# andres-quintela/manette

Hardware: AMD Instinct MI355X
Metric: env-steps/sec (ec x t_max frames per update) (higher is better)
Workload: dtype fp32

## Files before the change

manette_amd/csrc/net.hip:

```cpp
#include <string>
#include <vector>
#include <cmath>
#include <algorithm>
#include <tuple>

#include "gemm.h"
#include "jobs.h"
#include "trunk_fused.h"
#include "nips_bwd.h"
#include "dconv.h"
#include "nature_bwd.h"

namespace mt {

template <int C>
struct NipsArch {
  using Layers = std::tuple<ConvGeom<C, 16, 8, 4, 84, 84, false>, ConvGeom<16, 32, 4, 2, 20, 20, false>>;
  static constexpr int NCONV = 2;
  static constexpr unsigned POOL = 0;
  static constexpr int FLAT = 9 * 9 * 32;
  static constexpr int F = 256;
  static constexpr const char *FC = "fc3";
  static constexpr int FUSED_SLABS = FusedNips<C>::FC_SPLITS;
  static constexpr int FC_ROWS = 0;
// ... 918 lines not shown
                           float alpha) {
  using T = TileConvDgrad<G>;
  if constexpr (PhaseGeom<G>::OK) {
    constexpr int S2 = G::S * G::S;
    const int mp = cdiv(B * PhaseGeom<G>::HQ * PhaseGeom<G>::WQ, T::BM) * T::BM;
    return gemm_job<T>(LdConvBwdAPhase<G>{dY, mp, B}, LdConvBwdBPhase<G>{Wt, mp / T::BM},
                       EpMaskedPhase<G>{dX, Xact, mp, B, act, alpha}, S2 * mp, G::CIN, PhaseGeom<G>::KP, 1);
  } else {
    return gemm_job<T>(LdConvBwdA<G>{dY}, LdConvBwdB<G>{Wt}, EpMasked{dX, Xact, G::CIN, act, alpha},
                       B * G::H * G::W, G::CIN, G::KH * G::KW * G::COUT, 1);
  }
}

template <class G, class GJ>
static auto conv_dgrad_unpool_job(const float *dY, const float *Wt, const float *Pj, const uint8_t *argj,
                                  float *dactj, int B, int act, float alpha) {
  using T = TileConvDgrad<G>;
  static_assert(!PhaseGeom<G>::OK, "pooled inputs feed stride-1 convs (networks.py:206-225)");
  return gemm_job<T>(LdConvBwdA<G>{dY}, LdConvBwdB<G>{Wt}, EpMaskedUnpool<GJ>{dactj, Pj, argj, act, alpha},
                     B * G::H * G::W, G::CIN, G::KH * G::KW * G::COUT, 1);
}

#define MT_TRY(x)              \
  do {                         \
    int rc_ = (x);             \
    if (rc_ != MT_OK) return rc_; \
  } while (0)

template <class Ar, int I>
static const float *layer_out(float *ws, const WsLayout &L) {
  return ws + (pooled<Ar, I>() ? L.pool[I] : L.act[I]);
}

struct FwdExtras {
  const StackSrc *st = nullptr;
  uint32_t *sync = nullptr;
};

template <class Ar, int I = 0>
static int trunk_forward(const mt_net *n, const float *P, const void *x, int B, float *ws,
                         const WsLayout &L, hipStream_t s, const FwdExtras &ex = FwdExtras{}) {
  if constexpr (I < Ar::NCONV) {
    using G = LayerG<Ar, I>;
    const float *W = P + n->off_conv[I];
    if (I == 0 && ex.st && !nature_stacking<Ar>() && !frame_stacking<Ar>()) {
      set_error("the stacking conv1 is built for the NIPS, the gray NATURE and the frame (PWYX / LSTM) trunks");
      return MT_ERR_UNSUPPORTED;
    }
    if constexpr (I == 0 && frame_stacking<Ar>()) {
      if (ex.st) {
        if (!ex.sync || x != ex.st->out) {
          set_error("stacking conv1: the input must be the new state rows, with a counter region");
          return MT_ERR_ARG;
        }
        MT_TRY((launch_stack_conv1<G>(*ex.st, W, ws + L.pool[0], (uint8_t *)(ws + L.parg[0]), B, n->cfg.activation,
                                      n->cfg.alpha_leaky, ex.sync, s)));
        return trunk_forward<Ar, 1>(n, P, layer_out<Ar, 0>(ws, L), B, ws, L, s);
      }
    }
    if constexpr (I == 0 && nature_stacking<Ar>()) {
      if (ex.st) {
        if (!ex.sync) {
          set_error("nature chain: no counter region");
          return MT_ERR_ARG;
        }
        return launch_nature_chain<LayerG<Ar, 0>, LayerG<Ar, 1>, LayerG<Ar, 2>>(
            *ex.st, W, P + n->off_conv[1], P + n->off_conv[2], ws + L.act[0], ws + L.act[1], ws + L.act[2], B,
            n->cfg.activation, n->cfg.alpha_leaky, ex.sync, s);
      }
    }
    if constexpr ((G::S == 1 && G::SAME) || (Ar::NCONV == 3 && !G::SAME && G::CIN != 12))
      MT_TRY((conv_forward_direct<G, I == 0, pooled<Ar, I>()>(
          x, W, W + G::KK * G::COUT, ws + (pooled<Ar, I>() ? L.pool[I] : L.act[I]),
          pooled<Ar, I>() ? (uint8_t *)(ws + L.parg[I]) : nullptr, B, n->cfg.activation, n->cfg.alpha_leaky, s)));
    else if constexpr (pooled<Ar, I>())
      MT_TRY((conv_forward_pool<G, I == 0>(x, W, W + G::KK * G::COUT, ws + L.pool[I], (uint8_t *)(ws + L.parg[I]), B,
                                           n->cfg.activation, n->cfg.alpha_leaky, s)));
    else
      MT_TRY((conv_forward<G, I == 0>(x, W, W + G::KK * G::COUT, ws + L.act[I], B, n->cfg.activation,
                                      n->cfg.alpha_leaky, s)));
    return trunk_forward<Ar, I + 1>(n, P, layer_out<Ar, I>(ws, L), B, ws, L, s, ex);
  }
  return MT_OK;
}

struct NormOut {
  float *partials = nullptr;
  size_t n = 0;
};

template <class Ar, int I, class X = NoJob>
static int trunk_backward(const mt_net *n, const float *P, const uint8_t *obs, int B, float *ws,
                          const WsLayout &L, float *grad, hipStream_t s, SlabJob pending = SlabJob{},
                          const NormOut &no = NormOut{}, const X &extra = X{}) {
  using G = LayerG<Ar, I>;
  const int act = n->cfg.activation;
  const float al = n->cfg.alpha_leaky;
  const void *x = I == 0 ? (const void *)obs : (const void *)layer_out<Ar, (I > 0 ? I - 1 : 0)>(ws, L);
  if ((size_t)B * G::H * G::W * G::CIN >= ((size_t)1 << 31)) {
    set_error("batch %d too large for the conv %d weight gradient", B, I);
    return MT_ERR_ARG;
  }
  if ((size_t)B * G::OH * G::OW * G::COUT * 4 >= ((size_t)1 << 31) - 16) {
    set_error("batch %d too large for the conv %d input gradient", B, I);
    return MT_ERR_ARG;
  }
  const auto wg = conv_wgrad_jobs_sel<G, I == 0>(x, ws + L.dact[I], ws + (I % 2 ? L.wslab2 : L.wslab),
                                             grad + n->off_conv[I], B);
  if constexpr (I > 0) {
    constexpr int J = I - 1;
    using GJ = LayerG<Ar, J>;
    if constexpr (pooled<Ar, J>() && G::S == 1 && G::SAME && dconv_bwd_solo<G>()) {
      MT_TRY((conv_dgrad_unpool_solo<G, GJ>(ws + L.dact[I], P + n->off_conv[I], ws + L.pool[J],
                                           (const uint8_t *)(ws + L.parg[J]), ws + L.dact[J], B, act, al, s)));
      MT_TRY(launch_group(s, extra, wg.gemm, pending));
    } else if constexpr (stream_dx<G>()) {
      MT_TRY(launch_group(s, extra, DxStreamJob<G>{ws + L.dact[I], P + n->off_conv[I], ws + L.act[J], ws + L.dact[J], B,
                                            dx_stream_groups<G>(B), act, al},
                          wg.gemm, pending));
    } else if constexpr (pooled<Ar, J>()) {
      MT_TRY(launch_group(s, extra, conv_dgrad_unpool_job<G, GJ>(ws + L.dact[I], P + n->off_conv[I], ws + L.pool[J],
                                                           (const uint8_t *)(ws + L.parg[J]), ws + L.dact[J], B, act,
                                                           al),
                          wg.gemm, pending));
    } else {
      MT_TRY(launch_group(s, extra, conv_dgrad_job<G>(ws + L.dact[I], P + n->off_conv[I], ws + L.act[J], ws + L.dact[J], B,
                                               act, al),
                          wg.gemm, pending));
    }
    return trunk_backward<Ar, J>(n, P, obs, B, ws, L, grad, s, wg.sum, no);
  } else {
    MT_TRY(launch_group(s, extra, wg.gemm, pending));
    SlabJob last = wg.sum;
    if (no.partials && last.blocks() <= MT_NORM_PARTIALS / 2) {
      last.sq = no.partials;
      const size_t b0 = n->off_conv[0], b1 = b0 + last.n;
      SumsqJob rest{grad, no.n, last.blocks() ? b0 : 0, last.blocks() ? b1 : 0, no.partials + last.blocks(),
                    MT_NORM_PARTIALS - last.blocks()};
      return launch_group(s, last, rest);
    }
    MT_TRY(launch_group(s, last));
    if (no.partials)
      return launch_group(s, SumsqJob{grad, no.n, 0, 0, no.partials, MT_NORM_PARTIALS});
    return MT_OK;
  }
}

template <class Ar>
static int nips_conv_backward(const mt_net *n, const float *P, const uint8_t *obs, int B, float *ws,
                              const WsLayout &L, float *grad, hipStream_t s, const NormOut &no) {
  using J = NipsConvBwdJob;
  static_assert(LayerG<Ar, 0>::KK + 1 == 257 && LayerG<Ar, 1>::KK + 1 == 257, "slab rows");
  float *slab1 = ws + L.wslab, *slab2 = ws + L.wslab2;
  MT_TRY(launch_nips_conv_bwd(s, J{obs, ws + L.act[0], ws + L.dact[1], P + n->off_conv[1], ws + L.dact[0], slab1,
                                   slab2, B, n->cfg.activation, n->cfg.alpha_leaky}));
  SlabJob s1{slab1, B, (size_t)J::SLAB1, grad + n->off_conv[0]};
  SlabJob s2{slab2, (B + 1) / 2, (size_t)J::SLAB2, grad + n->off_conv[1]};
  if (!no.partials) return launch_group(s, s1, s2);
  s1.sq = no.partials;
  s2.sq = no.partials + s1.blocks();
  const int used = s1.blocks() + s2.blocks();
  static_assert(MT_NORM_PARTIALS >= 2 * ((257 * 16 / 4 + kSlabCols - 1) / kSlabCols + (257 * 32 / 4 + kSlabCols - 1) / kSlabCols),
                "norm partials");
  return launch_group(s, s1, s2,
                      SumsqJob{grad, no.n, n->off_conv[0], n->off_conv[1] + s2.n, no.partials + used,
                               MT_NORM_PARTIALS - used});
}

template <class Ar, int I = 0>
static void shift_rows(WsLayout &L, size_t row0) {
  if constexpr (I < Ar::NCONV) {
    using G = LayerG<Ar, I>;
    const size_t a = row0 * G::OH * G::OW * G::COUT;
    L.act[I] += a;
    L.dact[I] += a;
    if constexpr (pooled<Ar, I>()) {
      const size_t p = row0 * (G::OH / 2) * (G::OW / 2) * G::COUT;
      L.pool[I] += p;
      L.parg[I] += p / 4;
    }
    shift_rows<Ar, I + 1>(L, row0);
  }
}

struct ActRows {
  float *base;
  WsLayout L;
  size_t h_off;
};
template <class Ar>
static ActRows act_rows(const mt_net *n, float *ws, const WsLayout &L, const TrainRows *tr) {
  if (!tr) return ActRows{ws, L, L.H};
  ActRows a{tr->ws, ws_layout<Ar>(n, tr->rows), 0};
  a.h_off = a.L.H + (size_t)tr->row0 * Ar::F;
  shift_rows<Ar>(a.L, (size_t)tr->row0);
  return a;
}

template <class Ar>
static int forward_impl(const mt_net *n, const float *P, const uint8_t *obs, int B, float *ws,
                        float *v, float *pi, float *rep, const SampleArgs *smp, hipStream_t s,
                        const TrainRows *tr = nullptr, const hipEvent_t *marks = nullptr,
                        const StackSrc *st = nullptr) {
  const WsLayout L = ws_layout<Ar>(n, B);
  const ActRows A = act_rows<Ar>(n, ws, L, tr);
  if (marks) MT_HIP(hipEventRecord(marks[0], s));
  FwdExtras ex;
  ex.st = st;
  ex.sync = reinterpret_cast<uint32_t *>(ws + L.sync);
  MT_TRY((trunk_forward<Ar>(n, P, obs, B, A.base, A.L, s, ex)));
  const float *flat = layer_out<Ar, Ar::NCONV - 1>(A.base, A.L);
  const float *Wfc = P + n->off_fc;
  MT_TRY((launch_fc<Ar>(flat, B, Wfc, ws + L.fcslab, L.fc_splits, s)));
  if (marks) MT_HIP(hipEventRecord(marks[1], s));
  HeadParams hp = head_params(n, P);
  return launch_heads(B, s, ws + L.fcslab, L.fc_splits, B, Wfc + (size_t)Ar::FLAT * Ar::F, n->cfg.activation,
                      n->cfg.alpha_leaky, hp, n->cfg.softmax_temp, A.base + A.h_off, v, pi, rep,
                      smp ? *smp : SampleArgs{});
}

template <class Ar>
static int forward_infer_impl(const mt_net *n, const float *P, const uint8_t *obs, int B, float *ws,
                              float *v, float *pi, float *rep, const SampleArgs *smp, hipStream_t s,
                              const TrainRows *tr = nullptr, const StackSrc *st = nullptr,
                              const hipEvent_t *marks = nullptr) {
  if constexpr (Ar::FUSED_SLABS > 0) {
    constexpr int C = LayerG<Ar, 0>::CIN;
    using Fz = FusedNips<C>;
    const WsLayout L = ws_layout<Ar>(n, B);
    const ActRows A = act_rows<Ar>(n, ws, L, tr);
    const float *Wfc = P + n->off_fc;
    if (marks) MT_HIP(hipEventRecord(marks[0], s));
    MT_TRY((launch_nips_trunk<C>(obs, st, B, P + n->off_conv[0], P + n->off_conv[1], Wfc, n->cfg.activation,
                                 n->cfg.alpha_leaky, A.base + A.L.act[1], tr ? A.base + A.L.act[0] : nullptr,
                                 ws + L.fcslab, s)));
    MT_LAUNCHED();
    if (marks) MT_HIP(hipEventRecord(marks[1], s));
    HeadParams hp = head_params(n, P);
    return launch_heads(B, s, ws + L.fcslab, Fz::FC_SPLITS, B, Wfc + (size_t)Ar::FLAT * Ar::F, n->cfg.activation,
                        n->cfg.alpha_leaky, hp, n->cfg.softmax_temp, A.base + A.h_off, v, pi, rep,
                        smp ? *smp : SampleArgs{});
  } else {
    return forward_impl<Ar>(n, P, obs, B, ws, v, pi, rep, smp, s, tr, marks, st);
  }
}

template <class Ar>
static int forward_boot_impl(const mt_net *n, const float *P, const uint8_t *obs, int B, float *ws, hipStream_t s,
                             const StackSrc *st, uint32_t *advance, uint32_t advance_by) {
  const WsLayout L = ws_layout<Ar>(n, B);
  const float *Wfc = P + n->off_fc;
  if constexpr (Ar::FUSED_SLABS > 0) {
    constexpr int C = LayerG<Ar, 0>::CIN;
    return launch_nips_trunk<C>(obs, st, B, P + n->off_conv[0], P + n->off_conv[1], Wfc, n->cfg.activation,
                                n->cfg.alpha_leaky, ws + L.act[1], nullptr, ws + L.fcslab, s, advance, advance_by);
  } else {
    if (advance && Ar::FC_ROWS == 0) {
      set_error("sequence-base advance: row-split dense layers only");
      return MT_ERR_UNSUPPORTED;
    }
    FwdExtras ex;
    ex.st = st;
    ex.sync = reinterpret_cast<uint32_t *>(ws + L.sync);
    MT_TRY((trunk_forward<Ar>(n, P, obs, B, ws, L, s, ex)));
    return launch_fc<Ar>(layer_out<Ar, Ar::NCONV - 1>(ws, L), B, Wfc, ws + L.fcslab, L.fc_splits, s, advance,
                         advance_by);
  }
}

template <class Ar>
static int loss_bwd_launch(const mt_net *n, const float *P, int B, float *ws, const WsLayout &L, const float *pi,
                           const float *rep, const float *v, const int32_t *a_idx, const int32_t *r_idx,
                           const float *y, const float *adv, float beta, float *loss_terms, hipStream_t s,
                           const ReturnsSrc &rs = ReturnsSrc{}) {
  const float scale = 5.0f / (float)B;
  HeadParams hp = head_params(n, P);
  if (!launch_allowed()) return MT_OK;
  const size_t lds = (size_t)hp.nq * 16;
  if (lds > 150 * 1024) {
    set_error("loss: head region of %zu bytes exceeds the LDS", lds);
    return MT_ERR_ARG;
  }
  static bool attr_set = false;
  if (!attr_set && lds > 64 * 1024) {
    MT_HIP(hipFuncSetAttribute(reinterpret_cast<const void *>(&loss_bwd_kernel),
                               hipFuncAttributeMaxDynamicSharedMemorySize, 150 * 1024));
    attr_set = true;
  }
  hipLaunchKernelGGL(loss_bwd_kernel, dim3(B), dim3(256), lds, s, hp, ws + L.H, pi, rep, v, a_idx, r_idx, y, adv,
                     beta, scale, n->cfg.softmax_temp, n->cfg.activation, n->cfg.alpha_leaky, ws + L.dz, ws + L.dH,
                     loss_terms, rs);
  MT_LAUNCHED();
  return MT_OK;
}

template <class Ar>
static HeadWgradJob head_wgrad_job(const mt_net *n, int B, float *ws, const WsLayout &L, float *grad) {
  return HeadWgradJob{ws + L.H, ws + L.dz, B, Ar::F, n->cfg.num_actions, n->cfg.num_reps,
                      grad + n->off_critic, grad + n->off_actor, grad + n->off_rep};
}

template <class Ar>
static int heads_backward(const mt_net *n, const float *P, int B, float *ws, const WsLayout &L, const float *pi,
                          const float *rep, const float *v, const int32_t *a_idx, const int32_t *r_idx,
                          const float *y, const float *adv, float beta, float *grad, float *loss_terms,
                          hipStream_t s) {
  if (sizeof(float) * ((size_t)B + 4 * 64) > 160 * 1024) {
    set_error("batch %d exceeds the head-gradient LDS stage", B);
// ... 29 lines not shown
  const auto dx = gemm_job<TileDenseX>(LdRowMajor{ws + L.dH, Ar::F}, LdRowMajor{Wfc, Ar::F},
                                       EpMasked{ws + L.dact[K], flat, Ar::FLAT, act, al}, B, Ar::FLAT, Ar::F, 1);
  MT_TRY(launch_group(s, dx, dw, hw));
  if (g_win_on && g_win_index != kDenseBucketLaunches) {
    set_error("backward: the dense / head gradients completed after launch %d, not %d", g_win_index,
              kDenseBucketLaunches);
    return MT_ERR_UNSUPPORTED;
  }
  if constexpr (nips_fused_bwd<Ar>())
    if (B <= kNipsFusedBwdMaxRows) return nips_conv_backward<Ar>(n, P, obs, B, ws, L, grad, s, no);
  return trunk_backward<Ar, K>(n, P, obs, B, ws, L, grad, s, SlabJob{}, no);
}

}

#include "lstm.h"

using namespace mt;

#define MT_ARCH_SWITCH(net, ...)                                                   \
  do {                                                                              \
    const int arch_ = (net)->cfg.arch, d_ = (net)->cfg.depth;                       \
    if (arch_ == MT_ARCH_NIPS && d_ == 1) { using Ar = NipsArch<4>; __VA_ARGS__; }         \
    else if (arch_ == MT_ARCH_NIPS && d_ == 3) { using Ar = NipsArch<12>; __VA_ARGS__; }   \
    else if (arch_ == MT_ARCH_NATURE && d_ == 1) { using Ar = NatureArch<4>; __VA_ARGS__; } \
    else if (arch_ == MT_ARCH_NATURE && d_ == 3) { using Ar = NatureArch<12>; __VA_ARGS__; } \
    else if (arch_ == MT_ARCH_PWYX && d_ == 1) { using Ar = PwyxArch<4>; __VA_ARGS__; }     \
    else if (arch_ == MT_ARCH_PWYX && d_ == 3) { using Ar = PwyxArch<12>; __VA_ARGS__; }    \
    else if (arch_ == MT_ARCH_LSTM && d_ == 1) { using Ar = LstmArch<4>; __VA_ARGS__; }     \
    else if (arch_ == MT_ARCH_LSTM && d_ == 3) { using Ar = LstmArch<12>; __VA_ARGS__; }    \
    else { set_error("arch %d depth %d not built", arch_, d_); return MT_ERR_UNSUPPORTED; } \
  } while (0)

extern "C" int mt_net_create(const mt_net_config *cfg, mt_net **out) {
  MT_CHECK_ARG(cfg && out, "null argument");
  MT_CHECK_ARG(cfg->depth == 1 || cfg->depth == 3, "depth must be 1 or 3");
  MT_CHECK_ARG(cfg->num_actions >= 1 && cfg->num_actions <= 32, "num_actions out of range [1,32]");
  MT_CHECK_ARG(cfg->num_reps >= 1 && cfg->num_reps <= 31, "num_reps out of range [1,31]");
  MT_CHECK_ARG(cfg->activation == MT_ACT_RELU || cfg->activation == MT_ACT_LEAKY, "bad activation");
  MT_CHECK_ARG(cfg->softmax_temp > 0.f, "softmax_temp must be > 0");
  mt_net *n = new mt_net();
  n->cfg = *cfg;
  n->C = 4 * cfg->depth;
  n->O = 1 + cfg->num_actions + cfg->num_reps;
  const int arch = cfg->arch, d = cfg->depth;
  if (arch == MT_ARCH_NIPS && d == 1) build_layout<NipsArch<4>>(n);
  else if (arch == MT_ARCH_NIPS && d == 3) build_layout<NipsArch<12>>(n);
  else if (arch == MT_ARCH_NATURE && d == 1) build_layout<NatureArch<4>>(n);
  else if (arch == MT_ARCH_NATURE && d == 3) build_layout<NatureArch<12>>(n);
  else if (arch == MT_ARCH_PWYX && d == 1) build_layout<PwyxArch<4>>(n);
  else if (arch == MT_ARCH_PWYX && d == 3) build_layout<PwyxArch<12>>(n);
  else if (arch == MT_ARCH_LSTM && d == 1) build_layout_lstm<LstmArch<4>>(n);
  else if (arch == MT_ARCH_LSTM && d == 3) build_layout_lstm<LstmArch<12>>(n);
  else {
    delete n;
    set_error("arch %d not built into this library", arch);
    return MT_ERR_UNSUPPORTED;
  }
  *out = n;
  return MT_OK;
}

extern "C" void mt_net_destroy(mt_net *net) { delete net; }

extern "C" int mt_net_num_params(const mt_net *net, size_t *n) {
  MT_CHECK_ARG(net && n, "null argument");
  *n = net->nparams;
  return MT_OK;
}

extern "C" int mt_net_num_vars(const mt_net *net, int *n) {
  MT_CHECK_ARG(net && n, "null argument");
  *n = (int)net->vars.size();
  return MT_OK;
}

extern "C" int mt_net_var_info(const mt_net *net, int i, char *name, int name_len, int64_t *shape4,
                               int *ndim, size_t *offset, float *init_bound) {
  MT_CHECK_ARG(net, "null net");
  MT_CHECK_ARG(i >= 0 && i < (int)net->vars.size(), "var index %d out of range", i);
  const VarInfo &v = net->vars[i];
  if (name && name_len > 0) {
    std::strncpy(name, v.name.c_str(), name_len - 1);
    name[name_len - 1] = 0;
  }
  if (shape4)
    for (int k = 0; k < 4; ++k) shape4[k] = k < v.ndim ? v.shape[k] : 0;
  if (ndim) *ndim = v.ndim;
  if (offset) *offset = v.offset;
  if (init_bound) *init_bound = v.bound;
  return MT_OK;
}

extern "C" int mt_net_get_config(const mt_net *net, mt_net_config *cfg) {
  MT_CHECK_ARG(net && cfg, "null argument");
  *cfg = net->cfg;
  return MT_OK;
}

extern "C" int mt_net_feature_dim(const mt_net *net, int *f) {
  MT_CHECK_ARG(net && f, "null argument");
  *f = net->F;
  return MT_OK;
}

extern "C" int mt_net_workspace_bytes(const mt_net *net, int batch, size_t *bytes) {
  MT_CHECK_ARG(net && bytes, "null argument");
  MT_CHECK_ARG(batch >= 1, "batch must be >= 1");
  MT_ARCH_SWITCH(net, { *bytes = ws_layout<Ar>(net, batch).total * sizeof(float); });
  return MT_OK;
}

extern "C" int mt_net_backward_bucket_launches(const mt_net *net, int *launches) {
  MT_CHECK_ARG(net && launches, "null argument");
  MT_ARCH_SWITCH(net, {
    if constexpr (Ar::LSTM) {
      set_error("the LSTM backward is not bucketed");
      return MT_ERR_UNSUPPORTED;
    } else {
      *launches = kDenseBucketLaunches;
    }
  });
  return MT_OK;
}

template <class Ar, int I = 0>
static int ws_region(const WsLayout &L, int kind, int layer, size_t rows, size_t *offset, size_t *bytes) {
  if (kind == 4) {
    *offset = L.sync * sizeof(float);
    *bytes = (L.total - L.sync) * sizeof(float);
    return MT_OK;
  }
  if (kind == 2) {
    *offset = L.H * sizeof(float);
    *bytes = rows * Ar::F * sizeof(float);
    return MT_OK;
  }
  if constexpr (I < Ar::NCONV) {
    if (layer != I) return ws_region<Ar, I + 1>(L, kind, layer, rows, offset, bytes);
    using G = LayerG<Ar, I>;
    constexpr bool P = pooled<Ar, I>();
    const size_t px = P ? (size_t)(G::OH / 2) * (G::OW / 2) : (size_t)G::OH * G::OW;
    if (kind == 0) {
      *offset = (P ? L.pool[I] : L.act[I]) * sizeof(float);
      *bytes = rows * px * G::COUT * sizeof(float);
      return MT_OK;
    }
    if (kind == 1 && P) {
      *offset = L.parg[I] * sizeof(float);
      *bytes = rows * px * G::COUT;
      return MT_OK;
    }
    if (kind == 3) {
      *offset = L.dact[I] * sizeof(float);
      *bytes = rows * G::OH * G::OW * G::COUT * sizeof(float);
      return MT_OK;
    }
    set_error("conv layer %d has no region of kind %d", layer, kind);
    return MT_ERR_ARG;
  }
  set_error("no conv layer %d", layer);
  return MT_ERR_ARG;
}

template <class Ar>
static int ws_region_windows(const mt_net *net, int a, int kind, int layer, size_t *offset, size_t *bytes) {
  const WsLayout L = lstm_ws_layout<Ar>(net, a, nullptr);
  return ws_region<Ar>(L, kind, layer, kind == 2 ? (size_t)a : (size_t)a * Ar::STEPS, offset, bytes);
}

template <class Ar>
static int ws_region_frames(const mt_net *net, int E, int T, int kind, int layer, size_t *offset, size_t *bytes) {
  const LstmFrameWs X = lstm_frame_layout<Ar>(net, E, T);
  return ws_region<Ar>(X.L, kind, layer, kind == 2 ? (size_t)X.W : (size_t)X.R_max, offset, bytes);
}

extern "C" int mt_net_workspace_region(const mt_net *net, int layout, int a, int b, int kind, int layer,
                                       size_t *offset, size_t *bytes) {
  MT_CHECK_ARG(net && offset && bytes, "null argument");
  MT_CHECK_ARG(a >= 1 && (layout != 1 || b >= 1) && kind >= 0 && kind <= 4, "bad sizes or kind");
  MT_CHECK_ARG(kind != 4 || layout == 0, "the counter region (kind 4) is in the layout-0 workspace");
  MT_ARCH_SWITCH(net, {
    if (layout == 0) {
      if constexpr (Ar::LSTM) {
        set_error("layout 0 is the non-LSTM workspace");
        return MT_ERR_ARG;
      } else {
        return ws_region<Ar>(ws_layout<Ar>(net, a), kind, layer, (size_t)a, offset, bytes);
      }
    } else if (layout == 1 || layout == 2) {
      if constexpr (!Ar::LSTM) {
        set_error("layouts 1 and 2 are LSTM workspaces");
        return MT_ERR_ARG;
      } else {
        return layout == 1 ? ws_region_frames<Ar>(net, a, b, kind, layer, offset, bytes)
                           : ws_region_windows<Ar>(net, a, kind, layer, offset, bytes);
      }
    }
    set_error("layout %d", layout);
    return MT_ERR_ARG;
  });
  return MT_OK;
}

extern "C" int mt_forward(const mt_net *net, const float *params, const uint8_t *obs, int batch,
                          void *ws, size_t ws_bytes, float *v, float *pi, float *rep,
                          mt_stream_t stream) {
  return mt::forward_sample(net, params, obs, batch, ws, ws_bytes, v, pi, rep, nullptr, false,
                            (hipStream_t)stream);
}

template <class Ar>
static int trunk_infer_impl(const mt_net *n, const float *P, const uint8_t *obs, int B, float *ws, hipStream_t s,
                            const StackSrc *st = nullptr) {
  if constexpr (Ar::LSTM) {
    LstmWs X;
    const WsLayout L = lstm_ws_layout<Ar>(n, B, &X);
    const int rows = B * Ar::STEPS;
    MT_TRY((trunk_forward<Ar>(n, P, obs, rows, ws, L, s)));
    return launch_gemm<TileFc>(LdRowMajor{layer_out<Ar, Ar::NCONV - 1>(ws, L), Ar::FLAT},
                               LdColMajor{P + n->off_lstm, Ar::G4, -1}, EpSlab{ws + X.xg, rows, Ar::G4}, rows,
                               Ar::G4, Ar::FLAT, X.xg_splits, s);
  } else {
    const WsLayout L = ws_layout<Ar>(n, B);
    const float *Wfc = P + n->off_fc;
    if constexpr (Ar::FUSED_SLABS > 0) {
      constexpr int C = LayerG<Ar, 0>::CIN;
      MT_TRY((launch_nips_trunk<C>(obs, st, B, P + n->off_conv[0], P + n->off_conv[1], Wfc,
                                   n->cfg.activation, n->cfg.alpha_leaky, ws + L.act[1], nullptr, ws + L.fcslab, s)));
      MT_LAUNCHED();
      return MT_OK;
    } else {
      FwdExtras ex;
      ex.st = st;
      ex.sync = reinterpret_cast<uint32_t *>(ws + L.sync);
      MT_TRY((trunk_forward<Ar>(n, P, obs, B, ws, L, s, ex)));
      return launch_fc<Ar>(layer_out<Ar, Ar::NCONV - 1>(ws, L), B, Wfc, ws + L.fcslab, L.fc_splits, s);
    }
  }
}

extern "C" int mt_forward_trunk(const mt_net *net, const float *params, const uint8_t *obs, int batch, void *ws,
                                size_t ws_bytes, mt_stream_t stream) {
  MT_CHECK_ARG(net && params && obs && ws, "null argument");
  MT_CHECK_ARG(batch >= 1, "batch must be >= 1");
  MT_ARCH_SWITCH(net, {
    const WsLayout L = ws_layout<Ar>(net, batch);
    if (ws_bytes < L.total * sizeof(float)) {
      set_error("workspace %zu < %zu bytes", ws_bytes, L.total * sizeof(float));
      return MT_ERR_WORKSPACE;
    }
    return trunk_infer_impl<Ar>(net, params, obs, batch, (float *)ws, (hipStream_t)stream);
  });
  return MT_OK;
}

extern "C" int mt_forward_trunk_stacking(const mt_net *net, const float *params, const uint8_t *prev,
                                         const uint8_t *frames, const uint32_t *ready, uint32_t tag, uint8_t *out,
                                         int batch, void *ws, size_t ws_bytes, uint32_t *status,
                                         mt_stream_t stream) {
  MT_CHECK_ARG(net && params && prev && frames && ready && out && ws, "null argument");
  MT_CHECK_ARG(batch >= 1, "batch must be >= 1");
  StackSrc st{prev, frames, nullptr, out};
  st.ready = ready;
  st.tag = tag & 0x1fffffffu;
  st.status = status;
  MT_ARCH_SWITCH(net, {
    const WsLayout L = ws_layout<Ar>(net, batch);
    if (ws_bytes < L.total * sizeof(float)) {
      set_error("workspace %zu < %zu bytes", ws_bytes, L.total * sizeof(float));
      return MT_ERR_WORKSPACE;
    }
    if constexpr (Ar::LSTM) {
      set_error("stacking trunk: the NIPS, gray NATURE and PWYX archs (the LSTM steps: mt_lstm_step_forward)");
      return MT_ERR_UNSUPPORTED;
    } else {
      return trunk_infer_impl<Ar>(net, params, out, batch, (float *)ws, (hipStream_t)stream, &st);
    }
  });
  return MT_OK;
}

extern "C" int mt_forward_rows(const mt_net *net, const float *params, const uint8_t *obs, int batch, void *ws,
                               size_t ws_bytes, void *train_ws, size_t train_ws_bytes, int train_rows, int row0,
                               float *v, float *pi, float *rep, mt_stream_t stream) {
  MT_CHECK_ARG(train_ws, "null train workspace");
  const TrainRows tr{(float *)train_ws, train_ws_bytes, train_rows, row0};
  return mt::forward_sample(net, params, obs, batch, ws, ws_bytes, v, pi, rep, nullptr, true, (hipStream_t)stream,
                            &tr);
}

extern "C" int mt_forward_infer(const mt_net *net, const float *params, const uint8_t *obs, int batch,
                                void *ws, size_t ws_bytes, float *v, float *pi, float *rep,
                                mt_stream_t stream) {
  return mt::forward_sample(net, params, obs, batch, ws, ws_bytes, v, pi, rep, nullptr, true,
                            (hipStream_t)stream);
}

int mt::forward_sample(const mt_net *net, const float *params, const uint8_t *obs, int batch,
                       void *ws, size_t ws_bytes, float *v, float *pi, float *rep, const SampleArgs *smp,
                       bool infer, hipStream_t stream, const TrainRows *tr, const StackSrc *st,
                       const hipEvent_t *marks) {
  MT_CHECK_ARG(net && params && obs && ws && v && pi && rep, "null argument");
  MT_CHECK_ARG(!smp || !smp->counters || (smp->a_idx && smp->r_idx), "null sample buffer");
  MT_CHECK_ARG(batch >= 1, "batch must be >= 1");
  MT_ARCH_SWITCH(net, {
// ... 252 lines not shown
```

manette_amd/csrc/nips_bwd.h:

```cpp
#pragma once
#include "gemm.h"
#include "trunk_fused.h"

namespace mt {

struct NipsConvBwdJob {
  const uint8_t *X = nullptr;
  const float *act1 = nullptr, *dY2 = nullptr, *W2 = nullptr;
  float *dact1 = nullptr, *slab1 = nullptr, *slab2 = nullptr;
  int B = 0, act = 0;
  float alpha = 0.f;

  static constexpr int NT = 512;
  static constexpr int XROW = 24;
  static constexpr int XPLANE = 21 * XROW;
  static constexpr int X_BYTES = 64 * XPLANE;
  static constexpr int DS = 36;
  static constexpr int DY_FLOATS = 11 * 11 * DS;
  static constexpr int WS = 36;
  static constexpr int W2_FLOATS = 16 * 16 * WS;
  static constexpr int PS = 404;
  static constexpr int MAP_FLOATS = 16 * PS;
  static constexpr int SLAB1 = 257 * 16, SLAB2 = 257 * 32;
  static constexpr size_t LDS = X_BYTES + sizeof(float) * (DY_FLOATS + W2_FLOATS + 2 * MAP_FLOATS);
  static_assert(2 * sizeof(float) * (DY_FLOATS + MAP_FLOATS) <= LDS, "pair block stage");

  __host__ __device__ int pairs() const { return (B + 1) / 2; }
  __host__ __device__ int blocks() const { return B + pairs(); }

  struct DyAct {
    f32x4 yv[2], av[4];
  };
  __device__ __forceinline__ DyAct load_dy_act(int b) const {
    const int tid = threadIdx.x;
    const f32x4 *ys = reinterpret_cast<const f32x4 *>(dY2 + (size_t)b * 81 * 32);
    const f32x4 *as = reinterpret_cast<const f32x4 *>(act1 + (size_t)b * 400 * 16);
    DyAct d;
#pragma unroll
    for (int u = 0; u < 2; ++u) d.yv[u] = ys[min(tid + NT * u, 647)];
#pragma unroll
    for (int u = 0; u < 4; ++u) d.av[u] = as[min(tid + NT * u, 1599)];
    return d;
  }
  __device__ __forceinline__ void store_dy_act(const DyAct &d, float *dyp, float *a1t) const {
    const int tid = threadIdx.x;
    for (int i = tid; i < 121 * 8; i += NT) {
      const int p = i >> 3, Y = p / 11, Xc = p - 11 * Y;
      if (Y == 0 || Y == 10 || Xc == 0 || Xc == 10)
        *reinterpret_cast<f32x4 *>(dyp + p * DS + 4 * (i & 7)) = f32x4{0.f, 0.f, 0.f, 0.f};
    }
#pragma unroll
    for (int u = 0; u < 2; ++u) {
      const int i = tid + NT * u;
      if (i < 648) {
        const int p = i >> 3, oy = p / 9, ox = p - 9 * oy;
        *reinterpret_cast<f32x4 *>(dyp + ((oy + 1) * 11 + ox + 1) * DS + 4 * (i & 7)) = d.yv[u];
      }
    }
#pragma unroll
    for (int u = 0; u < 4; ++u) {
      const int i = tid + NT * u;
      if (i < 1600) {
        const int p = i >> 2, c = 4 * (i & 3);
#pragma unroll
        for (int e = 0; e < 4; ++e) a1t[(c + e) * PS + p] = d.av[u][e];
      }
    }
  }

  __device__ __forceinline__ void run(int bid, float *smem) const {
    if (bid < B)
      image_block(bid, smem);
    else
      pair_block(bid - B, smem);
  }

  __device__ __forceinline__ void image_block(int b, float *smem) const {
    float *dyp = smem;
    float *w2s = dyp + DY_FLOATS;
    float *a1t = w2s + W2_FLOATS;
    float *dat = a1t + MAP_FLOATS;
    uint8_t *xq = reinterpret_cast<uint8_t *>(dat + MAP_FLOATS);
    const int tid = threadIdx.x, lane = tid & 63, w = tid >> 6;
    const int r = lane & 15, g = lane >> 4;
    MT_PROBE_AT(3, b, 0);

    const uint4 *xs = reinterpret_cast<const uint4 *>(X + (size_t)b * 84 * 84 * 4);
    uint4 xv[4];
    {
      const int it = min(tid, 84 * 6 - 1), y = it / 6, jq = it - 6 * (it / 6);
#pragma unroll
      for (int v = 0; v < 4; ++v) xv[v] = xs[y * 21 + min(4 * jq + v, 20)];
    }
    const f32x4 *wsrc = reinterpret_cast<const f32x4 *>(W2);
    f32x4 wv[4];
#pragma unroll
    for (int u = 0; u < 4; ++u) wv[u] = wsrc[tid + NT * u];
    const DyAct da = load_dy_act(b);
    store_dy_act(da, dyp, a1t);
    if (tid < 84 * 6) {
      const int y = tid / 6, jq = tid - 6 * (tid / 6);
      uint8_t *row = xq + (y & 3) * 16 * XPLANE + (y >> 2) * XROW + 4 * jq;
#pragma unroll
      for (int p = 0; p < 4; ++p) {
        const uint32_t c0 = (&xv[0].x)[p], c1 = (&xv[1].x)[p], c2 = (&xv[2].x)[p], c3 = (&xv[3].x)[p];
#pragma unroll
        for (int ci = 0; ci < 4; ++ci) {
          const uint32_t d = ((c0 >> (8 * ci)) & 255u) | (((c1 >> (8 * ci)) & 255u) << 8) |
                             (((c2 >> (8 * ci)) & 255u) << 16) | ((c3 >> (8 * ci)) << 24);
          *reinterpret_cast<uint32_t *>(row + (p * 4 + ci) * XPLANE) = d;
        }
      }
    }
#pragma unroll
    for (int u = 0; u < 4; ++u) {
      const int i = tid + NT * u;
      *reinterpret_cast<f32x4 *>(w2s + (i >> 3) * WS + 4 * (i & 7)) = wv[u];
    }
    __syncthreads();
    MT_PROBE_AT(3, b, 1);

    {
      const int ph = w & 3, py = ph >> 1, px = ph & 1, t0 = 4 * (w >> 2);
      const int nt = w >> 2 ? 3 : 4;
      int off[4];
#pragma unroll
      for (int t = 0; t < 4; ++t) {
        const int q = min(16 * (t0 + t) + r, 99), qy = q / 10, qx = q - 10 * qy;
        off[t] = ((qy + 1) * 11 + qx + 1) * DS + 4 * g;
      }
      auto frags = [&](int kc, f32x4 &bf, f32x4 (&af)[4]) {
        const int ab = kc >> 1, a = ab >> 1, bb = ab & 1, co0 = (kc & 1) * 16;
        bf = *reinterpret_cast<const f32x4 *>(w2s + (((py + 2 * a) * 4 + px + 2 * bb) * 16 + r) * WS + co0 + 4 * g);
#pragma unroll
        for (int t = 0; t < 4; ++t) af[t] = *reinterpret_cast<const f32x4 *>(dyp + off[t] - (a * 11 + bb) * DS + co0);
      };
      f32x4 acc[4];
#pragma unroll
      for (int t = 0; t < 4; ++t) acc[t] = f32x4{0.f, 0.f, 0.f, 0.f};
      f32x4 bf, af[4];
      frags(0, bf, af);
#pragma unroll
      for (int kc = 0; kc < 8; ++kc) {
        f32x4 bn, an[4];
        if (kc + 1 < 8) frags(kc + 1, bn, an);
#pragma unroll
        for (int s = 0; s < 4; ++s)
#pragma unroll
          for (int t = 0; t < 4; ++t)
            if (t < nt) acc[t] = __builtin_amdgcn_mfma_f32_16x16x4f32(af[t][s], bf[s], acc[t], 0, 0, 0);
        if (kc + 1 < 8) {
          bf = bn;
#pragma unroll
          for (int t = 0; t < 4; ++t) af[t] = an[t];
        }
      }
#pragma unroll
      for (int t = 0; t < 4; ++t)
#pragma unroll
        for (int i = 0; i < 4; ++i) {
          const int q = 16 * (t0 + t) + 4 * g + i;
          if (q < 100) {
            const int qy = q / 10, qx = q - 10 * qy;
            const int p = (2 * qy + py) * 20 + 2 * qx + px;
            const float v = acc[t][i] * act_bwd(a1t[r * PS + p], act, alpha);
            dat[r * PS + p] = v;
            if (dact1) dact1[((size_t)b * 400 + p) * 16 + r] = v;
          }
        }
    }
    __syncthreads();
    MT_PROBE_AT(3, b, 2);

    {
      f32x4 acc[2] = {f32x4{0.f, 0.f, 0.f, 0.f}, f32x4{0.f, 0.f, 0.f, 0.f}};
      float db = 0.f;
      const uint8_t *pl = xq + ((w & 3) * 16 + r) * XPLANE + (w >> 2) * XROW;
      auto frag = [&](int kc, f32x4 &bf, uint32_t &u0, uint32_t &u1) {
        const int p0 = 16 * kc + 4 * g, oy = p0 / 20, ox0 = p0 - 20 * oy;
        bf = *reinterpret_cast<const f32x4 *>(dat + r * PS + p0);
        const uint32_t *src = reinterpret_cast<const uint32_t *>(pl + oy * XROW + ox0);
        u0 = src[0];
        u1 = __builtin_amdgcn_alignbyte(src[1], src[0], 1);
      };
      f32x4 bf;
      uint32_t u0, u1;
      frag(0, bf, u0, u1);
#pragma unroll 5
      for (int kc = 0; kc < 25; ++kc) {
        f32x4 bn;
        uint32_t n0, n1;
        frag(min(kc + 1, 24), bn, n0, n1);
#pragma unroll
        for (int s = 0; s < 4; ++s) {
          acc[0] = __builtin_amdgcn_mfma_f32_16x16x4f32((float)((u0 >> (8 * s)) & 255u), bf[s], acc[0], 0, 0, 0);
          acc[1] = __builtin_amdgcn_mfma_f32_16x16x4f32((float)((u1 >> (8 * s)) & 255u), bf[s], acc[1], 0, 0, 0);
        }
        db += (bf[0] + bf[1]) + (bf[2] + bf[3]);
        bf = bn;
        u0 = n0;
        u1 = n1;
      }
      const float sc = 1.0f / 255.0f;
      float *o = slab1 + (size_t)b * SLAB1;
#pragma unroll
      for (int mt = 0; mt < 2; ++mt)
#pragma unroll
        for (int i = 0; i < 4; ++i) o[(16 * (2 * w + mt) + 4 * g + i) * 16 + r] = acc[mt][i] * sc;
      db += __shfl_xor(db, 16, 64);
      db += __shfl_xor(db, 32, 64);
      if (w == 0 && lane < 16) o[256 * 16 + r] = db;
    }
    MT_PROBE_AT(3, b, 4);
  }

  __device__ __forceinline__ void pair_block(int q, float *smem) const {
    const int lane = threadIdx.x & 63, w = threadIdx.x >> 6;
    const int r = lane & 15, g = lane >> 4;
    const int nimg = 2 * q + 1 < B ? 2 : 1;
    float *dyp[2] = {smem, smem + DY_FLOATS + MAP_FLOATS};
    float *a1t[2] = {smem + DY_FLOATS, smem + 2 * DY_FLOATS + MAP_FLOATS};
    MT_PROBE_AT(3, B + q, 0);
    const DyAct d0 = load_dy_act(2 * q), d1 = load_dy_act(min(2 * q + 1, B - 1));
    store_dy_act(d0, dyp[0], a1t[0]);
    if (nimg == 2) store_dy_act(d1, dyp[1], a1t[1]);
    __syncthreads();
    MT_PROBE_AT(3, B + q, 1);
    f32x4 acc[2][2];
#pragma unroll
    for (int mt = 0; mt < 2; ++mt) acc[mt][0] = acc[mt][1] = f32x4{0.f, 0.f, 0.f, 0.f};
    float db0 = 0.f, db1 = 0.f;
    const int ky = w >> 1, kx0 = 2 * (w & 1);
    for (int im = 0; im < nimg; ++im) {
      const float *dy = dyp[im], *at = a1t[im];
#pragma unroll 3
      for (int j = 0; j < 21; ++j) {
        const int p = 4 * j + g, pc = min(p, 80), oy = pc / 9, ox = pc - 9 * oy;
        const int yo = p < 81 ? ((oy + 1) * 11 + ox + 1) * DS : 0;
        const float b0 = dy[yo + r], b1 = dy[yo + 16 + r];
        const float *ap = at + r * PS + (2 * oy + ky) * 20 + 2 * ox + kx0;
        const float a0 = ap[0], a1 = ap[1];
        acc[0][0] = __builtin_amdgcn_mfma_f32_16x16x4f32(a0, b0, acc[0][0], 0, 0, 0);
        acc[0][1] = __builtin_amdgcn_mfma_f32_16x16x4f32(a0, b1, acc[0][1], 0, 0, 0);
        acc[1][0] = __builtin_amdgcn_mfma_f32_16x16x4f32(a1, b0, acc[1][0], 0, 0, 0);
        acc[1][1] = __builtin_amdgcn_mfma_f32_16x16x4f32(a1, b1, acc[1][1], 0, 0, 0);
        db0 += b0;
        db1 += b1;
      }
    }
    float *o = slab2 + (size_t)q * SLAB2;
#pragma unroll
    for (int mt = 0; mt < 2; ++mt)
#pragma unroll
      for (int n = 0; n < 2; ++n)
#pragma unroll
        for (int i = 0; i < 4; ++i) o[(16 * (2 * w + mt) + 4 * g + i) * 32 + 16 * n + r] = acc[mt][n][i];
    db0 += __shfl_xor(db0, 16, 64);
    db0 += __shfl_xor(db0, 32, 64);
    db1 += __shfl_xor(db1, 16, 64);
    db1 += __shfl_xor(db1, 32, 64);
    if (w == 0 && lane < 16) {
      o[256 * 32 + r] = db0;
      o[256 * 32 + 16 + r] = db1;
    }
    MT_PROBE_AT(3, B + q, 4);
  }
};

__global__ __launch_bounds__(NipsConvBwdJob::NT) void nips_conv_bwd_kernel(NipsConvBwdJob j) {
  extern __shared__ __attribute__((aligned(16))) float smem[];
  j.run(blockIdx.x, smem);
}

inline int launch_nips_conv_bwd(hipStream_t s, const NipsConvBwdJob &j) {
  static_assert(NipsConvBwdJob::LDS <= 160 * 1024, "LDS budget");
  if (j.B <= 0 || !launch_allowed()) return MT_OK;
  static bool attr_set = false;
  if (!attr_set) {
    MT_HIP(hipFuncSetAttribute(reinterpret_cast<const void *>(&nips_conv_bwd_kernel),
                               hipFuncAttributeMaxDynamicSharedMemorySize, (int)NipsConvBwdJob::LDS));
    attr_set = true;
  }
  hipLaunchKernelGGL(nips_conv_bwd_kernel, dim3(j.blocks()), dim3(NipsConvBwdJob::NT), NipsConvBwdJob::LDS, s, j);
  MT_LAUNCHED();
  return MT_OK;
}

}
```

Before: 759,300.

## Restructure NIPS conv backward staging: register weights, drop dact1 store, repad LDS

The image block no longer stages W2 and the activation map in LDS. Each wave loads its weight fragments and the activation-mask values straight into registers, and the frame load is deferred so that half the waves transpose it into LDS after the MFMA products. The global write of conv layer 0's output gradient is dropped, and requests for that workspace region now return an error when the fused path applies. The pair block's LDS layout is changed to pixel-major rows padded to avoid bank conflicts, with incremental index updates replacing per-iteration divisions. This cuts LDS footprint, global writes and index arithmetic, at the cost of more registers and of no longer exposing dact1.

```diff
diff --git a/manette_amd/csrc/net.hip b/manette_amd/csrc/net.hip
--- a/manette_amd/csrc/net.hip
+++ b/manette_amd/csrc/net.hip
@@ -1094,8 +1094,8 @@
   using J = NipsConvBwdJob;
   static_assert(LayerG<Ar, 0>::KK + 1 == 257 && LayerG<Ar, 1>::KK + 1 == 257, "slab rows");
   float *slab1 = ws + L.wslab, *slab2 = ws + L.wslab2;
-  MT_TRY(launch_nips_conv_bwd(s, J{obs, ws + L.act[0], ws + L.dact[1], P + n->off_conv[1], ws + L.dact[0], slab1,
-                                   slab2, B, n->cfg.activation, n->cfg.alpha_leaky}));
+  MT_TRY(launch_nips_conv_bwd(s, J{obs, ws + L.act[0], ws + L.dact[1], P + n->off_conv[1], slab1, slab2, B,
+                                   n->cfg.activation, n->cfg.alpha_leaky}));
   SlabJob s1{slab1, B, (size_t)J::SLAB1, grad + n->off_conv[0]};
   SlabJob s2{slab2, (B + 1) / 2, (size_t)J::SLAB2, grad + n->off_conv[1]};
   if (!no.partials) return launch_group(s, s1, s2);
@@ -1431,6 +1431,12 @@
       return MT_OK;
     }
     if (kind == 3) {
+      if constexpr (nips_fused_bwd<Ar>() && I == 0)
+        if (rows <= (size_t)kNipsFusedBwdMaxRows) {
+          set_error("the fused NIPS conv backward (batch <= %d) does not store the gradient of conv layer 0's output",
+                    kNipsFusedBwdMaxRows);
+          return MT_ERR_ARG;
+        }
       *offset = L.dact[I] * sizeof(float);
       *bytes = rows * G::OH * G::OW * G::COUT * sizeof(float);
       return MT_OK;
diff --git a/manette_amd/csrc/nips_bwd.h b/manette_amd/csrc/nips_bwd.h
--- a/manette_amd/csrc/nips_bwd.h
+++ b/manette_amd/csrc/nips_bwd.h
@@ -1,4 +1,6 @@
 #pragma once
+#include <type_traits>
+
 #include "gemm.h"
 #include "trunk_fused.h"
 
@@ -7,7 +9,7 @@
 struct NipsConvBwdJob {
   const uint8_t *X = nullptr;
   const float *act1 = nullptr, *dY2 = nullptr, *W2 = nullptr;
-  float *dact1 = nullptr, *slab1 = nullptr, *slab2 = nullptr;
+  float *slab1 = nullptr, *slab2 = nullptr;
   int B = 0, act = 0;
   float alpha = 0.f;
 
@@ -17,56 +19,22 @@
   static constexpr int X_BYTES = 64 * XPLANE;
   static constexpr int DS = 36;
   static constexpr int DY_FLOATS = 11 * 11 * DS;
-  static constexpr int WS = 36;
-  static constexpr int W2_FLOATS = 16 * 16 * WS;
   static constexpr int PS = 404;
   static constexpr int MAP_FLOATS = 16 * PS;
+  static constexpr int AP = 24;
+  static constexpr int ACT_FLOATS = 400 * AP;
+  static constexpr int DP = 48;
+  static constexpr int DYP_FLOATS = 84 * DP;
   static constexpr int SLAB1 = 257 * 16, SLAB2 = 257 * 32;
-  static constexpr size_t LDS = X_BYTES + sizeof(float) * (DY_FLOATS + W2_FLOATS + 2 * MAP_FLOATS);
-  static_assert(2 * sizeof(float) * (DY_FLOATS + MAP_FLOATS) <= LDS, "pair block stage");
+  static constexpr size_t IMAGE_LDS = X_BYTES + sizeof(float) * (DY_FLOATS + MAP_FLOATS);
+  static constexpr size_t PAIR_LDS = 2 * sizeof(float) * (DYP_FLOATS + ACT_FLOATS);
+  static constexpr size_t LDS = IMAGE_LDS > PAIR_LDS ? IMAGE_LDS : PAIR_LDS;
+  static_assert(IMAGE_LDS <= LDS && PAIR_LDS <= LDS, "both block kinds fit");
+  static_assert(AP % 4 == 0 && DP % 4 == 0 && DS % 4 == 0 && (DY_FLOATS + MAP_FLOATS) % 4 == 0, "16-byte LDS rows");
+  static_assert((2 * AP) % 32 == 16 && DP % 32 == 16, "neighbouring pixels 16 banks apart");
 
   __host__ __device__ int pairs() const { return (B + 1) / 2; }
   __host__ __device__ int blocks() const { return B + pairs(); }
-
-  struct DyAct {
-    f32x4 yv[2], av[4];
-  };
-  __device__ __forceinline__ DyAct load_dy_act(int b) const {
-    const int tid = threadIdx.x;
-    const f32x4 *ys = reinterpret_cast<const f32x4 *>(dY2 + (size_t)b * 81 * 32);
-    const f32x4 *as = reinterpret_cast<const f32x4 *>(act1 + (size_t)b * 400 * 16);
-    DyAct d;
-#pragma unroll
-    for (int u = 0; u < 2; ++u) d.yv[u] = ys[min(tid + NT * u, 647)];
-#pragma unroll
-    for (int u = 0; u < 4; ++u) d.av[u] = as[min(tid + NT * u, 1599)];
-    return d;
-  }
-  __device__ __forceinline__ void store_dy_act(const DyAct &d, float *dyp, float *a1t) const {
-    const int tid = threadIdx.x;
-    for (int i = tid; i < 121 * 8; i += NT) {
-      const int p = i >> 3, Y = p / 11, Xc = p - 11 * Y;
-      if (Y == 0 || Y == 10 || Xc == 0 || Xc == 10)
-        *reinterpret_cast<f32x4 *>(dyp + p * DS + 4 * (i & 7)) = f32x4{0.f, 0.f, 0.f, 0.f};
-    }
-#pragma unroll
-    for (int u = 0; u < 2; ++u) {
-      const int i = tid + NT * u;
-      if (i < 648) {
-        const int p = i >> 3, oy = p / 9, ox = p - 9 * oy;
-        *reinterpret_cast<f32x4 *>(dyp + ((oy + 1) * 11 + ox + 1) * DS + 4 * (i & 7)) = d.yv[u];
-      }
-    }
-#pragma unroll
-    for (int u = 0; u < 4; ++u) {
-      const int i = tid + NT * u;
-      if (i < 1600) {
-        const int p = i >> 2, c = 4 * (i & 3);
-#pragma unroll
-        for (int e = 0; e < 4; ++e) a1t[(c + e) * PS + p] = d.av[u][e];
-      }
-    }
-  }
 
   __device__ __forceinline__ void run(int bid, float *smem) const {
     if (bid < B)
@@ -77,51 +45,76 @@
 
   __device__ __forceinline__ void image_block(int b, float *smem) const {
     float *dyp = smem;
-    float *w2s = dyp + DY_FLOATS;
-    float *a1t = w2s + W2_FLOATS;
-    float *dat = a1t + MAP_FLOATS;
+    float *dat = dyp + DY_FLOATS;
     uint8_t *xq = reinterpret_cast<uint8_t *>(dat + MAP_FLOATS);
-    const int tid = threadIdx.x, lane = tid & 63, w = tid >> 6;
+    const int tid = threadIdx.x, lane = tid & 63, w = __builtin_amdgcn_readfirstlane(tid >> 6);
     const int r = lane & 15, g = lane >> 4;
+    const int ph = w & 3, py = ph >> 1, px = ph & 1, t0 = 4 * (w >> 2);
     MT_PROBE_AT(3, b, 0);
 
+    f32x4 yv[2];
+    {
+      const f32x4 *ys = reinterpret_cast<const f32x4 *>(dY2 + (size_t)b * 81 * 32);
+#pragma unroll
+      for (int u = 0; u < 2; ++u) yv[u] = ys[min(tid + NT * u, 647)];
+    }
+    __builtin_amdgcn_sched_barrier(0);
+    f32x4 wq[8];
+#pragma unroll
+    for (int kc = 0; kc < 8; ++kc) {
+      const int ab = kc >> 1, a = ab >> 1, bb = ab & 1, co0 = (kc & 1) * 16;
+      wq[kc] = *reinterpret_cast<const f32x4 *>(W2 + (((py + 2 * a) * 4 + px + 2 * bb) * 16 + r) * 32 + co0 + 4 * g);
+    }
+    __builtin_amdgcn_sched_barrier(0);
+    float av[4][4];
+    auto load_mask = [&]() {
+      const float *as = act1 + (size_t)b * 400 * 16 + r;
+#pragma unroll
+      for (int t = 0; t < 4; ++t)
+#pragma unroll
+        for (int i = 0; i < 4; ++i) {
+          const int q = min(16 * (t0 + t) + 4 * g + i, 99), qy = q / 10, qx = q - 10 * qy;
+          av[t][i] = as[((2 * qy + py) * 20 + 2 * qx + px) * 16];
+        }
+    };
     const uint4 *xs = reinterpret_cast<const uint4 *>(X + (size_t)b * 84 * 84 * 4);
-    uint4 xv[4];
-    {
-      const int it = min(tid, 84 * 6 - 1), y = it / 6, jq = it - 6 * (it / 6);
-#pragma unroll
-      for (int v = 0; v < 4; ++v) xv[v] = xs[y * 21 + min(4 * jq + v, 20)];
-    }
-    const f32x4 *wsrc = reinterpret_cast<const f32x4 *>(W2);
-    f32x4 wv[4];
-#pragma unroll
-    for (int u = 0; u < 4; ++u) wv[u] = wsrc[tid + NT * u];
-    const DyAct da = load_dy_act(b);
-    store_dy_act(da, dyp, a1t);
-    if (tid < 84 * 6) {
-      const int y = tid / 6, jq = tid - 6 * (tid / 6);
-      uint8_t *row = xq + (y & 3) * 16 * XPLANE + (y >> 2) * XROW + 4 * jq;
-#pragma unroll
-      for (int p = 0; p < 4; ++p) {
-        const uint32_t c0 = (&xv[0].x)[p], c1 = (&xv[1].x)[p], c2 = (&xv[2].x)[p], c3 = (&xv[3].x)[p];
-#pragma unroll
-        for (int ci = 0; ci < 4; ++ci) {
-          const uint32_t d = ((c0 >> (8 * ci)) & 255u) | (((c1 >> (8 * ci)) & 255u) << 8) |
-                             (((c2 >> (8 * ci)) & 255u) << 16) | ((c3 >> (8 * ci)) << 24);
-          *reinterpret_cast<uint32_t *>(row + (p * 4 + ci) * XPLANE) = d;
-        }
-      }
-    }
-#pragma unroll
-    for (int u = 0; u < 4; ++u) {
+    constexpr int XU = 2;
+    const int it0 = tid - NT / 2;
+    const bool xw = w >> 2;
+    uint4 xv[XU][4];
+    auto load_frame = [&]() {
+      if (xw) {
+#pragma unroll
+        for (int u = 0; u < XU; ++u) {
+          const int it = min(it0 + NT / 2 * u, 84 * 6 - 1), y = it / 6, jq = it - 6 * (it / 6);
+#pragma unroll
+          for (int v = 0; v < 4; ++v) xv[u][v] = xs[y * 21 + min(4 * jq + v, 20)];
+        }
+      }
+    };
+
+    for (int i = tid; i < 121 * 8; i += NT) {
+      const int p = i >> 3, Y = p / 11, Xc = p - 11 * Y;
+      if (Y == 0 || Y == 10 || Xc == 0 || Xc == 10)
+        *reinterpret_cast<f32x4 *>(dyp + p * DS + 4 * (i & 7)) = f32x4{0.f, 0.f, 0.f, 0.f};
+    }
+#pragma unroll
+    for (int u = 0; u < 2; ++u) {
       const int i = tid + NT * u;
-      *reinterpret_cast<f32x4 *>(w2s + (i >> 3) * WS + 4 * (i & 7)) = wv[u];
+      if (i < 648) {
+        const int p = i >> 3, oy = p / 9, ox = p - 9 * oy;
+        *reinterpret_cast<f32x4 *>(dyp + ((oy + 1) * 11 + ox + 1) * DS + 4 * (i & 7)) = yv[u];
+      }
     }
     __syncthreads();
     MT_PROBE_AT(3, b, 1);
+    __builtin_amdgcn_sched_barrier(0);
+    load_mask();
+    __builtin_amdgcn_sched_barrier(0);
+    load_frame();
+    __builtin_amdgcn_sched_barrier(0);
 
     {
-      const int ph = w & 3, py = ph >> 1, px = ph & 1, t0 = 4 * (w >> 2);
       const int nt = w >> 2 ? 3 : 4;
       int off[4];
 #pragma unroll
@@ -129,30 +122,55 @@
         const int q = min(16 * (t0 + t) + r, 99), qy = q / 10, qx = q - 10 * qy;
         off[t] = ((qy + 1) * 11 + qx + 1) * DS + 4 * g;
       }
-      auto frags = [&](int kc, f32x4 &bf, f32x4 (&af)[4]) {
+      auto frags = [&](int kc, f32x4 (&af)[4]) {
         const int ab = kc >> 1, a = ab >> 1, bb = ab & 1, co0 = (kc & 1) * 16;
-        bf = *reinterpret_cast<const f32x4 *>(w2s + (((py + 2 * a) * 4 + px + 2 * bb) * 16 + r) * WS + co0 + 4 * g);
 #pragma unroll
         for (int t = 0; t < 4; ++t) af[t] = *reinterpret_cast<const f32x4 *>(dyp + off[t] - (a * 11 + bb) * DS + co0);
       };
       f32x4 acc[4];
 #pragma unroll
       for (int t = 0; t < 4; ++t) acc[t] = f32x4{0.f, 0.f, 0.f, 0.f};
-      f32x4 bf, af[4];
-      frags(0, bf, af);
-#pragma unroll
-      for (int kc = 0; kc < 8; ++kc) {
-        f32x4 bn, an[4];
-        if (kc + 1 < 8) frags(kc + 1, bn, an);
-#pragma unroll
-        for (int s = 0; s < 4; ++s)
-#pragma unroll
-          for (int t = 0; t < 4; ++t)
-            if (t < nt) acc[t] = __builtin_amdgcn_mfma_f32_16x16x4f32(af[t][s], bf[s], acc[t], 0, 0, 0);
-        if (kc + 1 < 8) {
-          bf = bn;
-#pragma unroll
-          for (int t = 0; t < 4; ++t) af[t] = an[t];
+      auto products = [&](auto ntc) {
+        constexpr int NTI = decltype(ntc)::value;
+        f32x4 af[4];
+        frags(0, af);
+#pragma unroll
+        for (int kc = 0; kc < 8; ++kc) {
+          f32x4 an[4];
+          if (kc + 1 < 8) frags(kc + 1, an);
+#pragma unroll
+          for (int s = 0; s < 4; ++s)
+#pragma unroll
+            for (int t = 0; t < NTI; ++t)
+              acc[t] = __builtin_amdgcn_mfma_f32_16x16x4f32(af[t][s], wq[kc][s], acc[t], 0, 0, 0);
+          if (kc + 1 < 8) {
+#pragma unroll
+            for (int t = 0; t < 4; ++t) af[t] = an[t];
+          }
+        }
+      };
+      if (nt == 4)
+        products(std::integral_constant<int, 4>{});
+      else
+        products(std::integral_constant<int, 3>{});
+      if (xw) {
+#pragma unroll
+        for (int u = 0; u < XU; ++u) {
+          const int it = it0 + NT / 2 * u;
+          if (it < 84 * 6) {
+            const int y = it / 6, jq = it - 6 * (it / 6);
+            uint8_t *row = xq + (y & 3) * 16 * XPLANE + (y >> 2) * XROW + 4 * jq;
+#pragma unroll
+            for (int p = 0; p < 4; ++p) {
+              const uint32_t c0 = (&xv[u][0].x)[p], c1 = (&xv[u][1].x)[p], c2 = (&xv[u][2].x)[p], c3 = (&xv[u][3].x)[p];
+#pragma unroll
+              for (int ci = 0; ci < 4; ++ci) {
+                const uint32_t d = ((c0 >> (8 * ci)) & 255u) | (((c1 >> (8 * ci)) & 255u) << 8) |
+                                   (((c2 >> (8 * ci)) & 255u) << 16) | ((c3 >> (8 * ci)) << 24);
+                *reinterpret_cast<uint32_t *>(row + (p * 4 + ci) * XPLANE) = d;
+              }
+            }
+          }
         }
       }
 #pragma unroll
@@ -163,9 +181,7 @@
           if (q < 100) {
             const int qy = q / 10, qx = q - 10 * qy;
             const int p = (2 * qy + py) * 20 + 2 * qx + px;
-            const float v = acc[t][i] * act_bwd(a1t[r * PS + p], act, alpha);
-            dat[r * PS + p] = v;
-            if (dact1) dact1[((size_t)b * 400 + p) * 16 + r] = v;
+            dat[r * PS + p] = acc[t][i] * act_bwd(av[t][i], act, alpha);
           }
         }
     }
@@ -214,16 +230,45 @@
     MT_PROBE_AT(3, b, 4);
   }
 
+  struct DyAct {
+    f32x4 yv[2], av[4];
+  };
+  __device__ __forceinline__ DyAct load_dy_act(int b) const {
+    const int tid = threadIdx.x;
+    const f32x4 *ys = reinterpret_cast<const f32x4 *>(dY2 + (size_t)b * 81 * 32);
+    const f32x4 *as = reinterpret_cast<const f32x4 *>(act1 + (size_t)b * 400 * 16);
+    DyAct d;
+#pragma unroll
+    for (int u = 0; u < 2; ++u) d.yv[u] = ys[min(tid + NT * u, 647)];
+#pragma unroll
+    for (int u = 0; u < 4; ++u) d.av[u] = as[min(tid + NT * u, 1599)];
+    return d;
+  }
+  __device__ __forceinline__ void store_dy_act(const DyAct &d, float *dy, float *at) const {
+    const int tid = threadIdx.x;
+    if (tid < 24)
+      *reinterpret_cast<f32x4 *>(dy + (81 + (tid >> 3)) * DP + 4 * (tid & 7)) = f32x4{0.f, 0.f, 0.f, 0.f};
+#pragma unroll
+    for (int u = 0; u < 2; ++u) {
+      const int i = tid + NT * u;
+      if (i < 648) *reinterpret_cast<f32x4 *>(dy + (i >> 3) * DP + 4 * (i & 7)) = d.yv[u];
+    }
+#pragma unroll
+    for (int u = 0; u < 4; ++u) {
+      const int i = tid + NT * u;
+      if (i < 1600) *reinterpret_cast<f32x4 *>(at + (i >> 2) * AP + 4 * (i & 3)) = d.av[u];
+    }
+  }
+
   __device__ __forceinline__ void pair_block(int q, float *smem) const {
     const int lane = threadIdx.x & 63, w = threadIdx.x >> 6;
     const int r = lane & 15, g = lane >> 4;
     const int nimg = 2 * q + 1 < B ? 2 : 1;
-    float *dyp[2] = {smem, smem + DY_FLOATS + MAP_FLOATS};
-    float *a1t[2] = {smem + DY_FLOATS, smem + 2 * DY_FLOATS + MAP_FLOATS};
+    constexpr int IMG = DYP_FLOATS + ACT_FLOATS;
     MT_PROBE_AT(3, B + q, 0);
     const DyAct d0 = load_dy_act(2 * q), d1 = load_dy_act(min(2 * q + 1, B - 1));
-    store_dy_act(d0, dyp[0], a1t[0]);
-    if (nimg == 2) store_dy_act(d1, dyp[1], a1t[1]);
+    store_dy_act(d0, smem, smem + DYP_FLOATS);
+    if (nimg == 2) store_dy_act(d1, smem + IMG, smem + IMG + DYP_FLOATS);
     __syncthreads();
     MT_PROBE_AT(3, B + q, 1);
     f32x4 acc[2][2];
@@ -231,21 +276,27 @@
     for (int mt = 0; mt < 2; ++mt) acc[mt][0] = acc[mt][1] = f32x4{0.f, 0.f, 0.f, 0.f};
     float db0 = 0.f, db1 = 0.f;
     const int ky = w >> 1, kx0 = 2 * (w & 1);
+    const int ao0 = (ky * 20 + 2 * g + kx0) * AP + r;
     for (int im = 0; im < nimg; ++im) {
-      const float *dy = dyp[im], *at = a1t[im];
-#pragma unroll 3
+      const float *dy = smem + im * IMG + g * DP + r, *at = smem + im * IMG + DYP_FLOATS;
+      int ao = ao0, ox = g;
+#pragma unroll
       for (int j = 0; j < 21; ++j) {
-        const int p = 4 * j + g, pc = min(p, 80), oy = pc / 9, ox = pc - 9 * oy;
-        const int yo = p < 81 ? ((oy + 1) * 11 + ox + 1) * DS : 0;
-        const float b0 = dy[yo + r], b1 = dy[yo + 16 + r];
-        const float *ap = at + r * PS + (2 * oy + ky) * 20 + 2 * ox + kx0;
-        const float a0 = ap[0], a1 = ap[1];
+        const float *ap = at + (j == 20 && g != 0 ? ao0 : ao);
+        const float b0 = dy[4 * j * DP], b1 = dy[4 * j * DP + 16];
+        const float a0 = ap[0], a1 = ap[AP];
         acc[0][0] = __builtin_amdgcn_mfma_f32_16x16x4f32(a0, b0, acc[0][0], 0, 0, 0);
         acc[0][1] = __builtin_amdgcn_mfma_f32_16x16x4f32(a0, b1, acc[0][1], 0, 0, 0);
         acc[1][0] = __builtin_amdgcn_mfma_f32_16x16x4f32(a1, b0, acc[1][0], 0, 0, 0);
         acc[1][1] = __builtin_amdgcn_mfma_f32_16x16x4f32(a1, b1, acc[1][1], 0, 0, 0);
         db0 += b0;
         db1 += b1;
+        ox += 4;
+        ao += 8 * AP;
+        if (ox >= 9) {
+          ox -= 9;
+          ao += (40 - 18) * AP;
+        }
       }
     }
     float *o = slab2 + (size_t)q * SLAB2;
```

Measured after the change: 760,000 (median of 4 runs). About the same (+0.1%).
